# mihikamd/DP-GSAT

Hardware: AMD Instinct MI355X
Metric: million edges/s (attn+sample+aggregate fwd+bwd) (higher is better)
Workload: dtype f32

## Files before the change

dp_gsat_amd/_lib.py:

```python
from __future__ import annotations

import ctypes
import os
from ctypes import c_char_p, c_double, c_float, c_int, c_int32, c_int64, c_size_t, c_uint64, c_void_p

import torch

_HERE = os.path.dirname(os.path.abspath(__file__))
LIB_PATH = os.path.join(_HERE, "libgsat_hip.so")

P, I64, I32, F32, F64, SZ, INT, U64 = c_void_p, c_int64, c_int32, c_float, c_double, c_size_t, c_int, c_uint64

SIGNATURES = {
    "gsat_abi_version": (INT, []),
    "gsat_seed_next": (INT, [P, P, P]),
    "gsat_last_error": (c_char_p, []),
    "gsat_csr_workspace_bytes": (SZ, [I64, I64]),
    "gsat_rev_workspace_bytes": (SZ, [I64]),
    "gsat_build_csr": (INT, [P, P, I64, I64, P, P, P, P, P, SZ, P]),
    "gsat_reverse_edge_perm": (INT, [P, I64, I64, P, P, P, SZ, P]),
    "gsat_reverse_edge_perm_csr": (INT, [P, P, P, P, P, P, P, P, I64, I64, P, P, P]),
    "gsat_segment_ptr": (INT, [P, I64, I64, P, P, P]),
    "gsat_gather_i64": (INT, [P, I64, P, I64, P, P]),
    "gsat_row_chunks_workspace_bytes": (SZ, [I64]),
# ... 29 lines not shown
    "gsat_bn_apply_fwd": (INT, [P, P, P, P, P, I64, I64, INT, P, F32, U64, P, P, P]),
    "gsat_bn_local_bwd_sums": (INT, [P, P, P, P, P, P, I64, I64, INT, F32, U64, P, P, P, P, P]),
    "gsat_bn_apply_bwd": (INT, [P, P, P, P, P, P, P, P, I64, P, I64, I64, INT, F32, U64, P, P, P, P]),
    "gsat_relu_dropout_fwd": (INT, [P, I64, I64, F32, U64, P, P, P]),
    "gsat_relu_dropout_bwd": (INT, [P, P, I64, I64, F32, P, P]),
    "gsat_colsum_workspace_floats": (SZ, [I64]),
    "gsat_colsum": (INT, [P, I64, I64, P, P, P]),
    "gsat_embsum_fwd": (INT, [P, P, INT, P, I64, I64, P, P]),
    "gsat_onehot_rows": (INT, [P, P, INT, I64, I64, P, P]),
    "gsat_gemm_workspace_floats": (SZ, [INT, I64, I64, I64]),
    "gsat_gemm_plan": (INT, [INT, INT, INT, I64, I64, I64, INT, INT, I64, P]),
    "gsat_gemm_f32": (INT, [INT, INT, I64, I64, I64, P, I64, P, I64, P, I64, P, INT, P, SZ, P]),
    "gsat_gemm_bf16x3": (INT, [INT, INT, I64, I64, I64, P, I64, P, I64, P, I64, P, INT, P, SZ, P]),
    "gsat_gemm_wgrad_plan": (INT, [I64, I64, I64, P]),
    "gsat_gemm_wgrad_x3": (INT, [I64, I64, I64, P, I64, P, I64, P, I64, INT, P, SZ, P]),
    "gsat_attn_fwd_workspace_bytes": (SZ, [P]),
    "gsat_attn_fwd_kind": (I32, [P]),
    "gsat_attn_bwd_workspace_bytes": (SZ, [P]),
    "gsat_attn_fwd": (INT, [P, P]),
    "gsat_attn_bwd": (INT, [P, P, P]),
    "gsat_instance_norm_fwd": (INT, [P, P, P, P, I64, I64, I64, P, P, P]),
    "gsat_instance_norm_bwd": (INT, [P, P, P, P, P, P, I64, I64, I64, P, P, P]),
    "gsat_philox_keep_mask": (INT, [U64, I32, I64, I64, F32, P, P]),
    "gsat_philox_noise": (INT, [U64, I64, P, P]),
    "gsat_sample_fwd": (INT, [P, P, INT, F32, F32, I64, P, P]),
    "gsat_sample_bwd": (INT, [P, P, F32, I64, P, P]),
    "gsat_gumbel_sigmoid_philox": (INT, [P, I64, F32, F32, U64, P, P, P]),
    "gsat_philox_gumbel_noise": (INT, [U64, I64, P, P]),
    "gsat_lift_fwd": (INT, [P, P, P, I64, P, P]),
    "gsat_lift_bwd": (INT, [P, P, P, P, P, P, P, P, I64, P, P]),
# ... 129 lines not shown
```

dp_gsat_amd/csrc/attn.hip:

```cpp
#include "common.h"
#include "attn_fused.h"
#include <cstdlib>

namespace gsat {

constexpr float IN_EPS = 1e-5f;
constexpr int SB = 256;
#ifndef GSAT_SB_LANES
#define GSAT_SB_LANES 16
#endif
constexpr int SB_LANES = GSAT_SB_LANES;
constexpr int SB_SLOTS = SB / SB_LANES;
constexpr int SB_RC = 2;

struct GemmWs { float* ptr; size_t floats; };
static int gemm_rm(hipStream_t stream, bool ta, bool tb, int64_t M, int64_t N, int64_t K, const float* A, int64_t lda, const float* B,
                   int64_t ldb, float beta, float* C, int64_t ldc, GemmWs ws = {nullptr, 0}, bool split_ok = false, SlabJob* defer = nullptr) {
    const char* env = getenv("GSAT_ATTN_BWD_SPLIT");
    const bool bwd_split = !(env && atoi(env) == 0);
    if (ta && !tb && split_ok && bwd_split) return gemm_wgrad(stream, M, N, K, A, lda, B, ldb, C, ldc, beta != 0.f, ws.ptr, ws.floats, defer);
    return gemm_f32(stream, ta, tb, M, N, K, A, lda, B, ldb, C, ldc, nullptr, beta != 0.f, ws.ptr, ws.floats, split_ok && bwd_split, defer);
}

template <bool EDGE>
struct PreAct {
    const float* P; const float* Q; const float* bias; const int32_t* src; const int32_t* dst; int C;
    __device__ __forceinline__ float4 load(int row, int c) const {
        float4 b = bias ? ld4(bias + c) : f4zero();
        float4 v;
        if (EDGE) {
            float4 p = ld4(P + (size_t)src[row] * C + c);
            float4 q = ld4(Q + (size_t)dst[row] * C + c);
            v = make_float4(p.x + q.x, p.y + q.y, p.z + q.z, p.w + q.w);
        } else {
            v = ld4(P + (size_t)row * C + c);
        }
// ... 845 lines not shown
    if (Z > 1) {
        const unsigned cb = (unsigned)ceil_div(G * C2, 256);
        k_zcombine<<<cb, 256, 0, stream>>>(zp1, a->seg_ptr, (int)G, Z, C2, 1, S1);
        k_zcombine<<<cb, 256, 0, stream>>>(zp2, a->seg_ptr, (int)G, Z, C2, 1, S2);
        k_zcombine<<<cb, 256, 0, stream>>>(zp3, a->seg_ptr, (int)G, Z, C2, 0, dw3p);
    }
    GSAT_LAUNCH_CHECK();
    if (!(merged && part_ok) && (rc = colsum(stream, dw3p, G, C2, gr->dW3, scratch))) return rc;
    if (Z > 1) {
        k_dh2<<<ew_blocks(M * (C2 / 4)), 256, 0, stream>>>(a->h2, a->b2, a->row_seg, mean2, rstd2, a->mask2, SeedRef{a->seed, a->seed_dev}, a->p_drop, a->training,
                                                           a->W3, dz, S1, S2, M, C2, dh2);
        GSAT_LAUNCH_CHECK();
    }
    if (dual_gemm_ok(1, M, C2, C1, C1)) {
        if ((rc = dual_gemm(stream, 1, M, C2, C1, C1, dh2, C2, a->a1, C1, a->W2, C1, da1, C1, 0, gr->dW2, C1, dws, dws_bytes))) return rc;
    } else {
        if ((rc = gemm_rm(stream, true, false, C2, C1, M, dh2, C2, a->a1, C1, 0.f, gr->dW2, C1, gws, true, &jobs[0]))) return rc;
        if ((rc = gemm_rm(stream, false, false, M, C1, C2, dh2, C2, a->W2, C1, 0.f, da1, C1, GemmWs{nullptr, 0}, true))) return rc;
    }
    if (Z == 1) {
        if (a->edge_mode) {
            PreAct<true> pre1{a->P, a->Q, a->b1, a->src, a->dst, C1};
            k_l1_bwd_stats<true, true><<<g1, SB, 0, stream>>>(da1, a->a1, a->seg_ptr, a->seg_order, sc, C1, S1p, S2p, pre1, mean1, rstd1);
        } else {
            PreAct<false> pre1{a->P, nullptr, a->b1, nullptr, nullptr, C1};
            k_l1_bwd_stats<true, false><<<g1, SB, 0, stream>>>(da1, a->a1, a->seg_ptr, a->seg_order, sc, C1, S1p, S2p, pre1, mean1, rstd1);
        }
    } else {
        k_l1_bwd_stats<false, false><<<g1, SB, 0, stream>>>(da1, a->a1, a->seg_ptr, a->seg_order, sc, C1, zp1, zp2);
    }
// ... 19 lines not shown
            if ((rc = dual_gemm(stream, 2, N, C1, H, H, dQ, C1, a->emb, H, a->W1 + H, 2 * H, gr->demb, H, 1, gr->dW1 + H, 2 * H, dws, dws_bytes))) return rc;
        } else {
        if ((rc = gemm_rm(stream, false, false, N, H, C1, dP, C1, a->W1, 2 * H, 0.f, gr->demb, H, GemmWs{nullptr, 0}, true))) return rc;
        if ((rc = gemm_rm(stream, false, false, N, H, C1, dQ, C1, a->W1 + H, 2 * H, 1.f, gr->demb, H, GemmWs{nullptr, 0}, true))) return rc;
        if ((rc = gemm_rm(stream, true, false, C1, H, N, dP, C1, a->emb, H, 0.f, gr->dW1, 2 * H, gws1, true, &jobs[1]))) return rc;
        if ((rc = gemm_rm(stream, true, false, C1, H, N, dQ, C1, a->emb, H, 0.f, gr->dW1 + H, 2 * H, gws1b, true, &jobs[2]))) return rc;
        }
    } else {
        if (Z > 1) {
            PreAct<false> pre{a->P, nullptr, a->b1, nullptr, nullptr, C1};
            k_dh1<false><<<ew_blocks(M * (C1 / 4)), 256, 0, stream>>>(pre, a->row_seg, mean1, rstd1, a->a1, sc, S1p, S2p, M, da1);
            GSAT_LAUNCH_CHECK();
        }
        if (dual_gemm_ok(2, N, C1, H, H)) {
            if ((rc = dual_gemm(stream, 2, N, C1, H, H, da1, C1, a->emb, H, a->W1, H, gr->demb, H, 0, gr->dW1, H, dws, dws_bytes))) return rc;
        } else {
        if ((rc = gemm_rm(stream, false, false, N, H, C1, da1, C1, a->W1, H, 0.f, gr->demb, H, GemmWs{nullptr, 0}, true))) return rc;
        if ((rc = gemm_rm(stream, true, false, C1, H, N, da1, C1, a->emb, H, 0.f, gr->dW1, H, gws1, true, &jobs[1]))) return rc;
        }
    }
    return slab_reduce_jobs(stream, jobs, 3);
}

int gsat_instance_norm_fwd(const float* x, const int32_t* seg_ptr, const int32_t* seg_order, const int32_t* row_seg, int64_t M,
                           int64_t G, int64_t C, float* y, float* stats, void* stream_) {
    hipStream_t stream = (hipStream_t)stream_;
    GSAT_REQUIRE(M >= 0 && G >= 0 && C > 0 && C % 4 == 0 && M < (1ll << 31), GSAT_ERR_UNSUPPORTED, "gsat_instance_norm_fwd: C must be a positive multiple of 4");
    if (M == 0 || G == 0) return GSAT_OK;
    GSAT_REQUIRE(x && seg_ptr && row_seg && y && stats, GSAT_ERR_ARG, "gsat_instance_norm_fwd: null pointer");
    float* mean = stats;
// ... 44 lines not shown
```

dp_gsat_amd/csrc/common.h:

```cpp
#pragma once
#include <cstring>
#include <cstdint>
#include <cstdio>
#include <cstdarg>
#include <hip/hip_runtime.h>

#include "../../include/gsat_hip.h"

namespace gsat {

void set_error(const char* fmt, ...);
const char* get_error();

#define GSAT_CHECK_HIP(expr)                                                                  \
    do {                                                                                      \
        hipError_t _e = (expr);                                                               \
        if (_e != hipSuccess) {                                                               \
            gsat::set_error("%s:%d: %s -> %s", __FILE__, __LINE__, #expr, hipGetErrorString(_e)); \
            return GSAT_ERR_HIP;                                                              \
        }                                                                                     \
    } while (0)

#define GSAT_REQUIRE(cond, code, ...)                                                         \
    do {                                                                                      \
// ... 23 lines not shown
    }
    bool ok() const { return base != nullptr && off <= cap; }
};

struct SlabJob { const float* ws; int nslab; size_t slab; int M, N; int64_t ldc; int accumulate; float* out; };
int gemm_f32(hipStream_t stream, bool a_t, bool b_t, int64_t M, int64_t N, int64_t K, const float* A, int64_t lda, const float* B,
             int64_t ldb, float* C, int64_t ldc, const float* bias, bool accumulate, float* ws, size_t ws_floats, bool allow_split = false,
             SlabJob* defer = nullptr);
int slab_reduce_jobs(hipStream_t stream, const SlabJob* jobs, int n);
size_t gemm_workspace_floats(int64_t M, int64_t N, int64_t K, bool reduce_rows);
struct WgradPlan { int eligible, S, rows; size_t ws_floats; };
WgradPlan wgrad_plan(int64_t Mo, int64_t No, int64_t K);
size_t gemm_wgrad_workspace_floats(int64_t Mo, int64_t No, int64_t K);
int gemm_wgrad(hipStream_t stream, int64_t Mo, int64_t No, int64_t K, const float* A, int64_t lda, const float* B, int64_t ldb, float* C,
               int64_t ldc, bool accumulate, float* ws, size_t ws_floats, SlabJob* defer = nullptr);

int aggr_sum_fwd_impl(hipStream_t stream, const float* x, const float* self_rows, const float* att, const float* edge_emb,
                      const int32_t* rowptr, const int32_t* col, const int32_t* eid, int64_t N, int64_t E, int64_t H, float self_coef,
                      float* out, const int32_t* chunk_ptr, float* partial);

#ifdef __HIPCC__
constexpr int WAVE = 64;

template <int CTRL> __device__ __forceinline__ float dpp_add(float v) {
    const int t = __builtin_amdgcn_update_dpp(0, __builtin_bit_cast(int, v), CTRL, 0xF, 0xF, true);
    return v + __builtin_bit_cast(float, t);
}

template <int WIDTH> __device__ __forceinline__ float group_sum(float v) {
    if constexpr ((WIDTH & (WIDTH - 1)) == 0) {
// ... 111 lines not shown
```

dp_gsat_amd/csrc/gemm.hip:

```cpp
#include "common.h"
#include "pna_math.h"
#include <cstdlib>

namespace gsat {

typedef float f32x16 __attribute__((ext_vector_type(16)));

constexpr int GK = 32, GT = 256;
constexpr int LD_KC = 129;
constexpr int LD_KM = 132;

struct StageKC { float4 v[4]; };
template <int ROWS>
__device__ __forceinline__ void load_kcontig(StageKC& s, const float* __restrict__ X, int64_t ld, int r0, int R, int k0, int K, int t) {
    const int kq = (t & 7) * 4;
#pragma unroll
    for (int p = 0; p < ROWS / 32; ++p) {
        const int r = r0 + (t >> 3) + 32 * p;
        s.v[p] = (r < R && k0 + kq < K) ? ld4(X + (size_t)r * ld + k0 + kq) : f4zero();
    }
}
template <int ROWS>
__device__ __forceinline__ void store_kcontig(const StageKC& s, float* __restrict__ L, int t) {
    const int kq = (t & 7) * 4;
// ... 13 lines not shown
#pragma unroll
    for (int p = 0; p < GK / KPP; ++p) {
        const int k = k0 + t / QPR + KPP * p;
        s.v[p] = (k < K && c0 + cq < Ccols) ? ld4(X + (size_t)k * ld + c0 + cq) : f4zero();
    }
}
template <int COLS>
__device__ __forceinline__ void store_kmajor(const StageKC& s, float* __restrict__ L, int t) {
    constexpr int QPR = COLS / 4, KPP = GT / QPR;
    const int cq = (t % QPR) * 4;
#pragma unroll
    for (int p = 0; p < GK / KPP; ++p) st4(L + (t / QPR + KPP * p) * LD_KM + cq, s.v[p]);
}

__device__ int GEMM_XCD_REMAP_ON = 1;
__device__ __forceinline__ void gemm_tile_coords(int& bx, int& by, int& bz) {
    const unsigned gx = gridDim.x, gy = gridDim.y, total = gx * gy * gridDim.z;
    const unsigned L = (blockIdx.z * gy + blockIdx.y) * gx + blockIdx.x;
    if (!GEMM_XCD_REMAP_ON) { bx = blockIdx.x; by = blockIdx.y; bz = blockIdx.z; return; }
    const unsigned q = total >> 3, r = total & 7, xcd = L & 7, i = L >> 3;
    const unsigned t = (xcd < r ? xcd * (q + 1) : r * (q + 1) + (xcd - r) * q) + i;
    bx = (int)(t % gx); by = (int)((t / gx) % gy); bz = (int)(t / (gx * gy));
}

template <bool A_T, bool B_T, int TM, int TN>
__global__ __launch_bounds__(GT) void k_gemm_f32(const float* __restrict__ A, int64_t lda, const float* __restrict__ B, int64_t ldb,
                                                 float* __restrict__ C, int64_t ldc, int M, int N, int K, int k_per_split,
                                                 const float* __restrict__ bias, int accumulate, size_t slab_stride) {
    constexpr int GM = 64 * TM, GN = 64 * TN;
    constexpr int LDA = A_T ? LD_KM : LD_KC, LDB = B_T ? LD_KC : LD_KM;
    constexpr int EP_LD = 36;
    static_assert(GK * LDA + GK * LDB >= 4 * 32 * EP_LD, "epilogue staging must fit in the operand images");
    __shared__ __attribute__((aligned(16))) float lds[GK * LDA + GK * LDB];
    float* const As = lds;
    float* const Bs = lds + GK * LDA;
    const int t = threadIdx.x, lane = t & 63, wave = t >> 6;
    const int wm = wave >> 1, wn = wave & 1;
// ... 415 lines not shown
                if (m0 + WS_ROWS <= M) {
#pragma unroll
                    for (int r = 0; r < 16; ++r) crow[(size_t)((r & 3) + 8 * (r >> 2)) * ldc] = acc[r] + bv;
                } else {
#pragma unroll
                    for (int r = 0; r < 16; ++r)
                        if (m0 + 4 * h + (r & 3) + 8 * (r >> 2) < M) crow[(size_t)((r & 3) + 8 * (r >> 2)) * ldc] = acc[r] + bv;
                }
            }
        }
        if (KS > 1) __syncthreads();
        float* tmp = cur; cur = nxt; nxt = tmp;
    }
}

template <bool B_T, int KSTEPS, int NQ>
__global__ __launch_bounds__(WS_THREADS, 2) void k_gemm_ws_x3(const float* __restrict__ A, int64_t lda, const float* __restrict__ B, int64_t ldb,
                                                             float* __restrict__ C, int64_t ldc, int M, int N, int K, int NB, int accumulate, int tiles) {
    extern __shared__ __attribute__((aligned(16))) unsigned char wx_lds[];
    const int RS = 2 * K + 16;
    const int PLANE = WS_ROWS * RS;
    unsigned char* const buf0 = wx_lds;
    unsigned char* const buf1 = wx_lds + 2 * PLANE;
    const int t = threadIdx.x, lane = t & 63, wave = t >> 6;
    const int cb = wave % NB, ks = wave / NB, KS = 8 / NB;
    const int c = lane & 31, h = lane >> 5;
    const int n0 = blockIdx.y * (NB * 32) + cb * 32;
    const int kw0 = ks * (KSTEPS * 16);
    bf16x8 bh[KSTEPS], bl[KSTEPS];
    {
        const int col = min(n0 + c, N - 1);
#pragma unroll
        for (int s_ = 0; s_ < KSTEPS; ++s_) {
            float v[8];
            const int k0 = kw0 + 16 * s_ + 8 * h;
            if (B_T) {
                const float4 v0 = ld4(B + (size_t)col * ldb + k0), v1 = ld4(B + (size_t)col * ldb + k0 + 4);
                v[0] = v0.x; v[1] = v0.y; v[2] = v0.z; v[3] = v0.w; v[4] = v1.x; v[5] = v1.y; v[6] = v1.z; v[7] = v1.w;
            } else {
#pragma unroll
                for (int j = 0; j < 8; ++j) v[j] = B[(size_t)(k0 + j) * ldb + col];
            }
            uint4 H = make_uint4(pack_bf16(v[0], v[1]), pack_bf16(v[2], v[3]), pack_bf16(v[4], v[5]), pack_bf16(v[6], v[7]));
            uint4 L = make_uint4(pack_bf16(v[0] - bf16_hi(v[0]), v[1] - bf16_hi(v[1])), pack_bf16(v[2] - bf16_hi(v[2]), v[3] - bf16_hi(v[3])),
                                 pack_bf16(v[4] - bf16_hi(v[4]), v[5] - bf16_hi(v[5])), pack_bf16(v[6] - bf16_hi(v[6]), v[7] - bf16_hi(v[7])));
            bh[s_] = *reinterpret_cast<bf16x8*>(&H);
            bl[s_] = *reinterpret_cast<bf16x8*>(&L);
        }
    }
    const int K4 = K >> 2;
    int srow[NQ], soff[NQ];
#pragma unroll
    for (int p = 0; p < NQ; ++p) {
        const int idx = t + p * WS_THREADS;
        srow[p] = idx / K4;
        soff[p] = 4 * (idx % K4);
    }
    float4 st[NQ];
    auto gload = [&](int tile) {
        const int m0 = tile * WS_ROWS;
#pragma unroll
        for (int p = 0; p < NQ; ++p) st[p] = ld4(A + (size_t)min(m0 + srow[p], M - 1) * lda + soff[p]);
    };
    auto lstore = [&](unsigned char* dst) {
#pragma unroll
        for (int p = 0; p < NQ; ++p) {
            const float4 v = st[p];
            const uint2 H = make_uint2(pack_bf16(v.x, v.y), pack_bf16(v.z, v.w));
            const uint2 L = make_uint2(pack_bf16(v.x - bf16_hi(v.x), v.y - bf16_hi(v.y)), pack_bf16(v.z - bf16_hi(v.z), v.w - bf16_hi(v.w)));
            *reinterpret_cast<uint2*>(dst + srow[p] * RS + soff[p] * 2) = H;
            *reinterpret_cast<uint2*>(dst + PLANE + srow[p] * RS + soff[p] * 2) = L;
        }
    };
    int tile = blockIdx.x;
    if (tile < tiles) { gload(tile); lstore(buf0); }
    __builtin_amdgcn_s_waitcnt(0x0F70);
    __syncthreads();
    unsigned char* cur = buf0;
    unsigned char* nxt = buf1;
    const bool col_ok = n0 + c < N;
    for (; tile < tiles; tile += gridDim.x) {
        const int ntile = tile + gridDim.x;
        if (ntile < tiles) gload(ntile);
        f32x16 acc;
#pragma unroll
        for (int r = 0; r < 16; ++r) acc[r] = 0.f;
        const unsigned char* arow = cur + c * RS + (kw0 + 8 * h) * 2;
#pragma unroll
        for (int s_ = 0; s_ < KSTEPS; ++s_) {
            const bf16x8 ah = *reinterpret_cast<const bf16x8*>(arow + 32 * s_);
            const bf16x8 al = *reinterpret_cast<const bf16x8*>(arow + PLANE + 32 * s_);
            acc = __builtin_amdgcn_mfma_f32_32x32x16_bf16(al, bl[s_], acc, 0, 0, 0);
            acc = __builtin_amdgcn_mfma_f32_32x32x16_bf16(al, bh[s_], acc, 0, 0, 0);
            acc = __builtin_amdgcn_mfma_f32_32x32x16_bf16(ah, bl[s_], acc, 0, 0, 0);
            acc = __builtin_amdgcn_mfma_f32_32x32x16_bf16(ah, bh[s_], acc, 0, 0, 0);
        }
        float* const xch = reinterpret_cast<float*>(cur);
        if (KS > 1) {
            __syncthreads();
            if (ks > 0) {
                float* part = xch + ((ks - 1) * NB + cb) * 1024;
#pragma unroll
                for (int r = 0; r < 16; ++r) part[r * 64 + lane] = acc[r];
            }
        }
        if (ntile < tiles) lstore(nxt);
        __syncthreads();
        if (ks == 0) {
            if (KS > 1) {
                for (int s2 = 1; s2 < KS; ++s2) {
                    const float* part = xch + ((s2 - 1) * NB + cb) * 1024;
#pragma unroll
                    for (int r = 0; r < 16; ++r) acc[r] += part[r * 64 + lane];
                }
            }
            const int m0 = tile * WS_ROWS;
            float* crow = C + (size_t)(m0 + 4 * h) * ldc + n0 + c;
            if (col_ok) {
#pragma unroll
                for (int r = 0; r < 16; ++r) {
                    const int rr = (r & 3) + 8 * (r >> 2);
                    if (m0 + 4 * h + rr < M) {
                        if (accumulate & 2) __builtin_nontemporal_store(acc[r], crow + (size_t)rr * ldc);
                        else crow[(size_t)rr * ldc] = (accumulate & 1) ? crow[(size_t)rr * ldc] + acc[r] : acc[r];
                    }
                }
            }
        }
        if (KS > 1) __syncthreads();
        unsigned char* tmp = cur; cur = nxt; nxt = tmp;
    }
}

__global__ void k_slab_reduce(const float* __restrict__ slabs, int nslab, size_t slab_stride, int M, int N, int64_t ldc,
                              int accumulate, float* __restrict__ out) {
    const int64_t i = (int64_t)blockIdx.x * blockDim.x + threadIdx.x;
    if (i >= (int64_t)M * N) return;
    const float* p0 = slabs + i;
    float a[8] = {0.f, 0.f, 0.f, 0.f, 0.f, 0.f, 0.f, 0.f};
    int s = 0;
    for (; s + 8 <= nslab; s += 8) {
#pragma unroll
        for (int j = 0; j < 8; ++j) a[j] += p0[(size_t)(s + j) * slab_stride];
    }
    for (int j = 0; s < nslab; ++s, ++j) a[j] += p0[(size_t)s * slab_stride];
    const float acc = ((a[0] + a[1]) + (a[2] + a[3])) + ((a[4] + a[5]) + (a[6] + a[7]));
// ... 148 lines not shown
    const int64_t NB = (N > 256 ? 256 : N) / 32;
    if (NB != 1 && NB != 2 && NB != 4 && NB != 8) return false;
    const int64_t KS = 8 / NB, Kw = K / KS;
    if (Kw % 16 != 0) return false;
    const int64_t st = Kw / 16;
    if (st != 2 && st != 4 && st != 8) return false;
    if ((KS - 1) * NB * 4096 > 2 * WS_ROWS * (2 * K + 16)) return false;
    *nb = (int)NB; *ksteps = (int)st;
    return true;
}
static bool wsx3_applicable(int64_t M, int64_t N, int64_t K) {
    static const int on = getenv("GSAT_GEMM_WSX3") ? atoi(getenv("GSAT_GEMM_WSX3")) : 1;
    int nb, st;
    return on && M >= 8192 && M < (1ll << 31) - 64 && wsx3_geometry(N, K, &nb, &st);
}
template <bool B_T, int KSTEPS, int NQ>
static int wsx3_launch(hipStream_t stream, dim3 grid, size_t lds, const float* A, int64_t lda, const float* B, int64_t ldb, float* C, int64_t ldc,
                       int M, int N, int K, int nb, int accumulate, int tiles) {
    static size_t allowed = 64 * 1024;
    if (lds > allowed) {
        GSAT_CHECK_HIP(hipFuncSetAttribute((const void*)k_gemm_ws_x3<B_T, KSTEPS, NQ>, hipFuncAttributeMaxDynamicSharedMemorySize, (int)lds));
        allowed = lds;
    }
    k_gemm_ws_x3<B_T, KSTEPS, NQ><<<grid, WS_THREADS, lds, stream>>>(A, lda, B, ldb, C, ldc, M, N, K, nb, accumulate, tiles);
    GSAT_LAUNCH_CHECK();
    return GSAT_OK;
}
static int gemm_wsx3(hipStream_t stream, bool b_t, int64_t M, int64_t N, int64_t K, const float* A, int64_t lda, const float* B, int64_t ldb,
                     float* C, int64_t ldc, bool accumulate, int nb, int st) {
    const int tiles = (int)ceil_div(M, WS_ROWS);
    const size_t lds = (size_t)4 * WS_ROWS * (2 * K + 16);
    const int nq = (int)(K / 64);
    const int per_cu = (2 * lds <= 150 * 1024 && st * 8 + nq * 9 <= 84) ? 2 : 1;
    const int chunks = (int)ceil_div(N, 256);
    const dim3 grid((unsigned)std::min<int64_t>(tiles, std::max<int64_t>(1, (int64_t)256 * per_cu / chunks)), (unsigned)chunks);
    static const int nt_mode = getenv("GSAT_GEMM_NT") ? atoi(getenv("GSAT_GEMM_NT")) : 1;
    const int acc_flag = (accumulate ? 1 : 0) | ((nt_mode && !accumulate && (size_t)M * N * 4 >= ((size_t)64 << 20)) ? 2 : 0);
#define XGO(BT, S, Q) return wsx3_launch<BT, S, Q>(stream, grid, lds, A, lda, B, ldb, C, ldc, (int)M, (int)N, (int)K, nb, acc_flag, tiles)
#define XQ(BT, S) do { switch (nq) { case 1: XGO(BT, S, 1); case 2: XGO(BT, S, 2); case 4: XGO(BT, S, 4); case 8: XGO(BT, S, 8); default: break; } } while (0)
#define XS(BT) do { switch (st) { case 2: XQ(BT, 2); break; case 4: XQ(BT, 4); break; default: XQ(BT, 8); break; } } while (0)
    if (b_t) XS(true); else XS(false);
#undef XS
#undef XQ
#undef XGO
    GSAT_REQUIRE(false, GSAT_ERR_UNSUPPORTED, "gemm_wsx3: K = %lld is not 64, 128, 256 or 512", (long long)K);
}

enum { GEMM_TILE_F32 = 0, GEMM_TILE_X3 = 1, GEMM_WS_F32 = 2, GEMM_WS_X3 = 3 };
struct GemmPlan {
    int family;
    int tm, tn;
    int splits;
// ... 106 lines not shown
    }
    for (int q = m; q <= 4; ++q) J.first[q] = blocks;
    if (!blocks) return GSAT_OK;
    if (wide == 4) k_slab_reduce_jobs<16><<<blocks, 256, 0, stream>>>(J);
    else if (wide == 2) k_slab_reduce_jobs<8><<<blocks, 256, 0, stream>>>(J);
    else k_slab_reduce_jobs<4><<<blocks, 256, 0, stream>>>(J);
    GSAT_LAUNCH_CHECK();
    return GSAT_OK;
}

constexpr int WG_T = 512, WG_TILE = 128;
constexpr int WG_PLANE = (GK / 8) * WG_TILE * 16;
constexpr int WG_BUF = 4 * WG_PLANE;
constexpr int WG_MIN_SLABS = 8;

__global__ __launch_bounds__(WG_T) void k_wgrad_x3(const float* A, int64_t lda, const float* B, int64_t ldb, float* ws, int Mo, int No, int K,
                                                   int rows_per) {
    constexpr int EP_LD = 36;
    static_assert(2 * WG_BUF >= 8 * 32 * EP_LD * 4, "epilogue staging must fit in the operand planes");
    __shared__ __attribute__((aligned(16))) unsigned char lds[2 * WG_BUF];
    const int t = threadIdx.x, lane = t & 63, wave = t >> 6;
    int bx, by, bz;
    gemm_tile_coords(bx, by, bz);
    const int m0 = by * WG_TILE, n0 = bx * WG_TILE;
    const int kbeg = bz * rows_per, kend = min(K, kbeg + rows_per);
    const int nslab = (kend - kbeg + GK - 1) / GK;
    const int ts = t & 255, cp = (ts & 63) * 2, k8 = ts >> 6;
    const bool stage_b = t >= 256;
    const float* const src = stage_b ? B + n0 + cp : A + m0 + cp;
    const int64_t ld = stage_b ? ldb : lda;
    const int plane0 = stage_b ? 2 * WG_PLANE : 0;
    auto gload = [&](StageKM& s, int slab) {
        const int kb = kbeg + slab * GK + k8 * 8;
#pragma unroll
        for (int j = 0; j < 8; ++j) s.v[j] = *reinterpret_cast<const float2*>(src + (size_t)min(kb + j, kend - 1) * ld);
    };
    auto lstore = [&](StageKM& s, int slab, unsigned char* buf) {
        const int kb = kbeg + slab * GK + k8 * 8;
// ... 64 lines not shown
    const int prow = lane >> 3, pcol = (lane & 7) * 4;
#pragma unroll
    for (int j = 0; j < 2; ++j) {
#pragma unroll
        for (int r = 0; r < 16; ++r) patch[((r & 3) + 8 * (r >> 2) + 4 * kh) * EP_LD + r32] = acc[j][r];
        __builtin_amdgcn_wave_barrier();
        const int col = n0 + wn * 64 + j * 32 + pcol;
#pragma unroll
        for (int p = 0; p < 4; ++p) {
            const int rr = prow + 8 * p;
            st4(Cb + (size_t)(m0 + wm * 32 + rr) * No + col, ld4(patch + rr * EP_LD + pcol));
        }
        __builtin_amdgcn_wave_barrier();
    }
}

static int device_cus() {
    static const int n = [] {
        int dev = 0, v = 0;
        if (hipGetDevice(&dev) != hipSuccess || hipDeviceGetAttribute(&v, hipDeviceAttributeMultiprocessorCount, dev) != hipSuccess || v <= 0) {
            (void)hipGetLastError();
            v = 256;
        }
        return v;
    }();
    return n;
}

WgradPlan wgrad_plan(int64_t Mo, int64_t No, int64_t K) {
    WgradPlan p{};
// ... 18 lines not shown

int gemm_wgrad(hipStream_t stream, int64_t Mo, int64_t No, int64_t K, const float* A, int64_t lda, const float* B, int64_t ldb, float* C,
               int64_t ldc, bool accumulate, float* ws, size_t ws_floats, SlabJob* defer) {
    const WgradPlan p = wgrad_plan(Mo, No, K);
    if (!p.eligible) return gemm_f32(stream, true, false, Mo, No, K, A, lda, B, ldb, C, ldc, nullptr, accumulate, ws, ws_floats, true, defer);
    if (defer) defer->nslab = 0;
    xcd_switch_once();
    GSAT_REQUIRE(A && B && C && lda >= Mo && ldb >= No && ldc >= No && lda % 4 == 0 && ldb % 4 == 0 && ldc % 4 == 0, GSAT_ERR_ARG, "gemm_wgrad: bad argument");
    GSAT_REQUIRE(((uintptr_t)A % 16 == 0) && ((uintptr_t)B % 16 == 0) && ((uintptr_t)C % 16 == 0) && ((uintptr_t)ws % 16 == 0), GSAT_ERR_ARG,
                 "gemm_wgrad: operands, output and workspace must be 16-byte aligned");
    GSAT_REQUIRE(ws && ws_floats >= p.ws_floats, GSAT_ERR_WORKSPACE, "gemm_wgrad: workspace too small");
    const dim3 grid((unsigned)(No / WG_TILE), (unsigned)(Mo / WG_TILE), (unsigned)p.S);
    k_wgrad_x3<<<grid, WG_T, 0, stream>>>(A, lda, B, ldb, ws, (int)Mo, (int)No, (int)K, p.rows);
    GSAT_LAUNCH_CHECK();
    const SlabJob job{ws, p.S, (size_t)Mo * No, (int)Mo, (int)No, ldc, accumulate ? 1 : 0, C};
    if (defer) { *defer = job; return GSAT_OK; }
    return slab_reduce_jobs(stream, &job, 1);
}

int pna_post_fwd(hipStream_t stream, const PnaVirt& pv, int64_t Nrows, const float* W, int64_t ldw, const float* bias, int64_t Ho, float* out, int64_t ldo) {
    const int64_t K = (int64_t)pv.NAGG * 2 * pv.H;
    GSAT_REQUIRE(pv.H % 32 == 0 && Ho % 4 == 0 && ldw % 4 == 0 && ldo % 4 == 0 && Nrows < (1ll << 31), GSAT_ERR_UNSUPPORTED, "gsat_pna_post_fwd: H must be a multiple of 32, Ho of 4");
    GSAT_REQUIRE(((uintptr_t)W % 16 == 0) && ((uintptr_t)out % 16 == 0) && (!bias || (uintptr_t)bias % 16 == 0) && ((uintptr_t)pv.x % 16 == 0) && ((uintptr_t)pv.aggj % 16 == 0),
                 GSAT_ERR_ARG, "gsat_pna_post_fwd: operands must be 16-byte aligned");
    if (Nrows <= 0 || Ho <= 0) return GSAT_OK;
    xcd_switch_once();
    const int tn = Ho > 64 ? 2 : 1;
    dim3 grid((unsigned)ceil_div(Ho, 64 * tn), (unsigned)ceil_div(Nrows, 128), 1);
    if (tn == 2) k_gemm_bf16x3<false, true, 2, 2, 1><<<grid, GT, 0, stream>>>(nullptr, 0, W, ldw, out, ldo, (int)Nrows, (int)Ho, (int)K, (int)K, bias, 0, 0, pv);
    else k_gemm_bf16x3<false, true, 2, 1, 1><<<grid, GT, 0, stream>>>(nullptr, 0, W, ldw, out, ldo, (int)Nrows, (int)Ho, (int)K, (int)K, bias, 0, 0, pv);
// ... 79 lines not shown

int gsat_gemm_wgrad_plan(int64_t Mo, int64_t No, int64_t K, int32_t* plan) {
    GSAT_REQUIRE(plan && Mo > 0 && No > 0 && K > 0, GSAT_ERR_ARG, "gsat_gemm_wgrad_plan: bad argument");
    const WgradPlan p = wgrad_plan(Mo, No, K);
    GSAT_REQUIRE(p.ws_floats <= (size_t)INT32_MAX, GSAT_ERR_UNSUPPORTED, "gsat_gemm_wgrad_plan: workspace of %zu floats does not fit int32", p.ws_floats);
    const int32_t v[4] = {p.eligible, p.S, p.rows, (int32_t)p.ws_floats};
    memcpy(plan, v, sizeof(v));
    return GSAT_OK;
}

int gsat_gemm_wgrad_x3(int64_t Mo, int64_t No, int64_t K, const float* A, int64_t lda, const float* B, int64_t ldb, float* C, int64_t ldc,
                       int accumulate, float* workspace, size_t workspace_floats, void* stream) {
    return gemm_wgrad((hipStream_t)stream, Mo, No, K, A, lda, B, ldb, C, ldc, accumulate != 0, workspace, workspace_floats);
}

int gsat_gemm_plan(int allow_split, int a_t, int b_t, int64_t M, int64_t N, int64_t K, int has_bias, int accumulate, int64_t ldb, int32_t* plan) {
    GSAT_REQUIRE(plan && M > 0 && N > 0 && K > 0, GSAT_ERR_ARG, "gsat_gemm_plan: bad argument");
    GSAT_REQUIRE(ldb % 4 == 0 && (a_t ? M % 4 == 0 : K % 4 == 0) && (b_t ? K % 4 == 0 : N % 4 == 0), GSAT_ERR_UNSUPPORTED,
                 "gsat_gemm_plan: contiguous extents and leading dimensions must be multiples of 4 (M=%lld N=%lld K=%lld)", (long long)M, (long long)N, (long long)K);
    const GemmPlan p = gemm_plan(allow_split != 0, a_t != 0, b_t != 0, M, N, K, has_bias != 0, accumulate != 0, ldb);
    GSAT_REQUIRE(!(has_bias && p.splits > 1), GSAT_ERR_UNSUPPORTED, "gsat_gemm_plan: bias with split-K");
    const int32_t v[8] = {p.family, p.tm, p.tn, p.splits, p.reduce, p.nb, p.kr, p.nq};
    memcpy(plan, v, sizeof(v));
    return GSAT_OK;
}

}
```

include/gsat_hip.h:

```cpp
#ifndef GSAT_HIP_H
#define GSAT_HIP_H

#include <stddef.h>
#include <stdint.h>

#ifdef __cplusplus
extern "C" {
#endif

#define GSAT_ABI_VERSION 4

#define GSAT_OK 0
#define GSAT_ERR_HIP (-1)
#define GSAT_ERR_ARG (-2)
#define GSAT_ERR_WORKSPACE (-3)
#define GSAT_ERR_UNSUPPORTED (-4)
#define GSAT_ERR_BLAS (-5)

int gsat_abi_version(void);

int gsat_seed_next(uint64_t* state, uint64_t* out, void* stream);
const char* gsat_last_error(void);


// ... 156 lines not shown
                     void* stream);


size_t gsat_gemm_workspace_floats(int a_t, int64_t M, int64_t N, int64_t K);
int gsat_gemm_plan(int allow_split, int a_t, int b_t, int64_t M, int64_t N, int64_t K, int has_bias, int accumulate,
                   int64_t ldb, int32_t* plan);
int gsat_gemm_f32(int a_t, int b_t, int64_t M, int64_t N, int64_t K, const float* A, int64_t lda,
                  const float* B, int64_t ldb, float* C, int64_t ldc, const float* bias, int accumulate,
                  float* workspace, size_t workspace_floats, void* stream);
int gsat_gemm_bf16x3(int a_t, int b_t, int64_t M, int64_t N, int64_t K, const float* A, int64_t lda,
                     const float* B, int64_t ldb, float* C, int64_t ldc, const float* bias, int accumulate,
                     float* workspace, size_t workspace_floats, void* stream);
int gsat_gemm_wgrad_plan(int64_t Mo, int64_t No, int64_t K, int32_t* plan);
int gsat_gemm_wgrad_x3(int64_t Mo, int64_t No, int64_t K, const float* A, int64_t lda, const float* B, int64_t ldb,
                       float* C, int64_t ldc, int accumulate, float* workspace, size_t workspace_floats, void* stream);


typedef struct gsat_attn_args {
    int64_t M, N, G;
    int32_t H, C1, C2;
    int32_t edge_mode;
    int32_t training;
    float p_drop;
    uint64_t seed;
    const int32_t* src;
    const int32_t* dst;
    const int32_t* seg_ptr;
    const int32_t* seg_order;
    const int32_t* row_seg;
    const float *W1, *b1, *W2, *b2, *W3, *b3;
// ... 229 lines not shown
```

Baseline: 132.5.

## Co-schedule weight-grad and data-grad GEMMs in one paired kernel launch

```diff
diff --git a/dp_gsat_amd/_lib.py b/dp_gsat_amd/_lib.py
--- a/dp_gsat_amd/_lib.py
+++ b/dp_gsat_amd/_lib.py
@@ -67,6 +67,8 @@
     "gsat_gemm_bf16x3": (INT, [INT, INT, I64, I64, I64, P, I64, P, I64, P, I64, P, INT, P, SZ, P]),
     "gsat_gemm_wgrad_plan": (INT, [I64, I64, I64, P]),
     "gsat_gemm_wgrad_x3": (INT, [I64, I64, I64, P, I64, P, I64, P, I64, INT, P, SZ, P]),
+    "gsat_gemm_pair_plan": (INT, [I64, I64, I64, I64, P]),
+    "gsat_gemm_pair_x3": (INT, [I64, I64, I64, I64, P, I64, P, I64, P, I64, P, I64, P, I64, INT, P, SZ, P]),
     "gsat_attn_fwd_workspace_bytes": (SZ, [P]),
     "gsat_attn_fwd_kind": (I32, [P]),
     "gsat_attn_bwd_workspace_bytes": (SZ, [P]),
diff --git a/dp_gsat_amd/csrc/attn.hip b/dp_gsat_amd/csrc/attn.hip
--- a/dp_gsat_amd/csrc/attn.hip
+++ b/dp_gsat_amd/csrc/attn.hip
@@ -20,6 +20,10 @@
     const bool bwd_split = !(env && atoi(env) == 0);
     if (ta && !tb && split_ok && bwd_split) return gemm_wgrad(stream, M, N, K, A, lda, B, ldb, C, ldc, beta != 0.f, ws.ptr, ws.floats, defer);
     return gemm_f32(stream, ta, tb, M, N, K, A, lda, B, ldb, C, ldc, nullptr, beta != 0.f, ws.ptr, ws.floats, split_ok && bwd_split, defer);
+}
+static bool pair_ok(int64_t R, int64_t Cg, int64_t Co, int64_t Cy) {
+    const char* env = getenv("GSAT_ATTN_BWD_SPLIT");
+    return !(env && atoi(env) == 0) && gemm_pair_plan(R, Cg, Co, Cy).paired;
 }
 
 template <bool EDGE>
@@ -895,6 +899,8 @@
     }
     if (dual_gemm_ok(1, M, C2, C1, C1)) {
         if ((rc = dual_gemm(stream, 1, M, C2, C1, C1, dh2, C2, a->a1, C1, a->W2, C1, da1, C1, 0, gr->dW2, C1, dws, dws_bytes))) return rc;
+    } else if (pair_ok(M, C2, C1, C1)) {
+        if ((rc = gemm_pair_x3(stream, M, C2, C1, C1, dh2, C2, a->W2, C1, da1, C1, a->a1, C1, gr->dW2, C1, false, gws.ptr, gws.floats, &jobs[0]))) return rc;
     } else {
         if ((rc = gemm_rm(stream, true, false, C2, C1, M, dh2, C2, a->a1, C1, 0.f, gr->dW2, C1, gws, true, &jobs[0]))) return rc;
         if ((rc = gemm_rm(stream, false, false, M, C1, C2, dh2, C2, a->W2, C1, 0.f, da1, C1, GemmWs{nullptr, 0}, true))) return rc;
@@ -944,6 +950,8 @@
         }
         if (dual_gemm_ok(2, N, C1, H, H)) {
             if ((rc = dual_gemm(stream, 2, N, C1, H, H, da1, C1, a->emb, H, a->W1, H, gr->demb, H, 0, gr->dW1, H, dws, dws_bytes))) return rc;
+        } else if (pair_ok(N, C1, H, H)) {
+            if ((rc = gemm_pair_x3(stream, N, C1, H, H, da1, C1, a->W1, H, gr->demb, H, a->emb, H, gr->dW1, H, false, gws1.ptr, gws1.floats, &jobs[1]))) return rc;
         } else {
         if ((rc = gemm_rm(stream, false, false, N, H, C1, da1, C1, a->W1, H, 0.f, gr->demb, H, GemmWs{nullptr, 0}, true))) return rc;
         if ((rc = gemm_rm(stream, true, false, C1, H, N, da1, C1, a->emb, H, 0.f, gr->dW1, H, gws1, true, &jobs[1]))) return rc;
diff --git a/dp_gsat_amd/csrc/common.h b/dp_gsat_amd/csrc/common.h
--- a/dp_gsat_amd/csrc/common.h
+++ b/dp_gsat_amd/csrc/common.h
@@ -61,6 +61,11 @@
 size_t gemm_wgrad_workspace_floats(int64_t Mo, int64_t No, int64_t K);
 int gemm_wgrad(hipStream_t stream, int64_t Mo, int64_t No, int64_t K, const float* A, int64_t lda, const float* B, int64_t ldb, float* C,
                int64_t ldc, bool accumulate, float* ws, size_t ws_floats, SlabJob* defer = nullptr);
+struct PairPlan { int paired, wgrad_blocks, dgrad_blocks, lds_bytes; };
+PairPlan gemm_pair_plan(int64_t R, int64_t Cg, int64_t Co, int64_t Cy);
+int gemm_pair_x3(hipStream_t stream, int64_t R, int64_t Cg, int64_t Co, int64_t Cy, const float* G, int64_t ldg, const float* W, int64_t ldw,
+                 float* OUT, int64_t ldo, const float* Y, int64_t ldy, float* DW, int64_t lddw, bool accumulate, float* ws, size_t ws_floats,
+                 SlabJob* defer = nullptr);
 
 int aggr_sum_fwd_impl(hipStream_t stream, const float* x, const float* self_rows, const float* att, const float* edge_emb,
                       const int32_t* rowptr, const int32_t* col, const int32_t* eid, int64_t N, int64_t E, int64_t H, float self_coef,
diff --git a/dp_gsat_amd/csrc/gemm.hip b/dp_gsat_amd/csrc/gemm.hip
--- a/dp_gsat_amd/csrc/gemm.hip
+++ b/dp_gsat_amd/csrc/gemm.hip
@@ -51,13 +51,17 @@
 }
 
 __device__ int GEMM_XCD_REMAP_ON = 1;
+__device__ __forceinline__ void gemm_tile_coords(unsigned L, unsigned gx, unsigned gy, unsigned gz, int& bx, int& by, int& bz) {
+    const unsigned total = gx * gy * gz;
+    unsigned t = L;
+    if (GEMM_XCD_REMAP_ON) {
+        const unsigned q = total >> 3, r = total & 7, xcd = L & 7, i = L >> 3;
+        t = (xcd < r ? xcd * (q + 1) : r * (q + 1) + (xcd - r) * q) + i;
+    }
+    bx = (int)(t % gx); by = (int)((t / gx) % gy); bz = (int)(t / (gx * gy));
+}
 __device__ __forceinline__ void gemm_tile_coords(int& bx, int& by, int& bz) {
-    const unsigned gx = gridDim.x, gy = gridDim.y, total = gx * gy * gridDim.z;
-    const unsigned L = (blockIdx.z * gy + blockIdx.y) * gx + blockIdx.x;
-    if (!GEMM_XCD_REMAP_ON) { bx = blockIdx.x; by = blockIdx.y; bz = blockIdx.z; return; }
-    const unsigned q = total >> 3, r = total & 7, xcd = L & 7, i = L >> 3;
-    const unsigned t = (xcd < r ? xcd * (q + 1) : r * (q + 1) + (xcd - r) * q) + i;
-    bx = (int)(t % gx); by = (int)((t / gx) % gy); bz = (int)(t / (gx * gy));
+    gemm_tile_coords((blockIdx.z * gridDim.y + blockIdx.y) * gridDim.x + blockIdx.x, gridDim.x, gridDim.y, gridDim.z, bx, by, bz);
 }
 
 template <bool A_T, bool B_T, int TM, int TN>
@@ -503,10 +507,11 @@
     }
 }
 
-template <bool B_T, int KSTEPS, int NQ>
-__global__ __launch_bounds__(WS_THREADS, 2) void k_gemm_ws_x3(const float* __restrict__ A, int64_t lda, const float* __restrict__ B, int64_t ldb,
-                                                             float* __restrict__ C, int64_t ldc, int M, int N, int K, int NB, int accumulate, int tiles) {
-    extern __shared__ __attribute__((aligned(16))) unsigned char wx_lds[];
+template <bool B_T, int KSTEPS, int NQ, bool KFIX = false>
+__device__ __forceinline__ void gemm_ws_x3_body(unsigned char* wx_lds, int bx, int by, int gx, const float* __restrict__ A, int64_t lda,
+                                                const float* __restrict__ B, int64_t ldb, float* __restrict__ C, int64_t ldc, int M, int N, int K_,
+                                                int NB_, int accumulate, int tiles) {
+    const int K = KFIX ? 64 * NQ : K_, NB = KFIX ? 2 * KSTEPS / NQ : NB_;
     const int RS = 2 * K + 16;
     const int PLANE = WS_ROWS * RS;
     unsigned char* const buf0 = wx_lds;
@@ -514,7 +519,7 @@
     const int t = threadIdx.x, lane = t & 63, wave = t >> 6;
     const int cb = wave % NB, ks = wave / NB, KS = 8 / NB;
     const int c = lane & 31, h = lane >> 5;
-    const int n0 = blockIdx.y * (NB * 32) + cb * 32;
+    const int n0 = by * (NB * 32) + cb * 32;
     const int kw0 = ks * (KSTEPS * 16);
     bf16x8 bh[KSTEPS], bl[KSTEPS];
     {
@@ -545,31 +550,38 @@
         srow[p] = idx / K4;
         soff[p] = 4 * (idx % K4);
     }
-    float4 st[NQ];
-    auto gload = [&](int tile) {
+    constexpr bool HALVES = KFIX && NQ == 4 && KSTEPS == 8;
+    constexpr int NS = HALVES ? NQ / 2 : NQ;
+    float4 st[NS];
+    auto gload = [&](int tile, int half = 0) {
         const int m0 = tile * WS_ROWS;
 #pragma unroll
-        for (int p = 0; p < NQ; ++p) st[p] = ld4(A + (size_t)min(m0 + srow[p], M - 1) * lda + soff[p]);
+        for (int p = 0; p < NS; ++p)
+            st[p] = ld4(A + (size_t)min(m0 + srow[p + half * NS], M - 1) * lda + soff[p + half * NS]);
     };
-    auto lstore = [&](unsigned char* dst) {
-#pragma unroll
-        for (int p = 0; p < NQ; ++p) {
+    auto lstore = [&](unsigned char* dst, int half = 0) {
+#pragma unroll
+        for (int p = 0; p < NS; ++p) {
             const float4 v = st[p];
+            const int o = srow[p + half * NS] * RS + soff[p + half * NS] * 2;
             const uint2 H = make_uint2(pack_bf16(v.x, v.y), pack_bf16(v.z, v.w));
             const uint2 L = make_uint2(pack_bf16(v.x - bf16_hi(v.x), v.y - bf16_hi(v.y)), pack_bf16(v.z - bf16_hi(v.z), v.w - bf16_hi(v.w)));
-            *reinterpret_cast<uint2*>(dst + srow[p] * RS + soff[p] * 2) = H;
-            *reinterpret_cast<uint2*>(dst + PLANE + srow[p] * RS + soff[p] * 2) = L;
+            *reinterpret_cast<uint2*>(dst + o) = H;
+            *reinterpret_cast<uint2*>(dst + PLANE + o) = L;
         }
     };
-    int tile = blockIdx.x;
-    if (tile < tiles) { gload(tile); lstore(buf0); }
+    int tile = bx;
+    if (tile < tiles) {
+        gload(tile); lstore(buf0);
+        if (HALVES) { gload(tile, 1); lstore(buf0, 1); }
+    }
     __builtin_amdgcn_s_waitcnt(0x0F70);
     __syncthreads();
     unsigned char* cur = buf0;
     unsigned char* nxt = buf1;
     const bool col_ok = n0 + c < N;
-    for (; tile < tiles; tile += gridDim.x) {
-        const int ntile = tile + gridDim.x;
+    for (; tile < tiles; tile += gx) {
+        const int ntile = tile + gx;
         if (ntile < tiles) gload(ntile);
         f32x16 acc;
 #pragma unroll
@@ -583,6 +595,7 @@
             acc = __builtin_amdgcn_mfma_f32_32x32x16_bf16(al, bh[s_], acc, 0, 0, 0);
             acc = __builtin_amdgcn_mfma_f32_32x32x16_bf16(ah, bl[s_], acc, 0, 0, 0);
             acc = __builtin_amdgcn_mfma_f32_32x32x16_bf16(ah, bh[s_], acc, 0, 0, 0);
+            if (HALVES && s_ == KSTEPS / 2 - 1 && ntile < tiles) { lstore(nxt); gload(ntile, 1); }
         }
         float* const xch = reinterpret_cast<float*>(cur);
         if (KS > 1) {
@@ -593,7 +606,7 @@
                 for (int r = 0; r < 16; ++r) part[r * 64 + lane] = acc[r];
             }
         }
-        if (ntile < tiles) lstore(nxt);
+        if (ntile < tiles) lstore(nxt, HALVES ? 1 : 0);
         __syncthreads();
         if (ks == 0) {
             if (KS > 1) {
@@ -619,6 +632,12 @@
         if (KS > 1) __syncthreads();
         unsigned char* tmp = cur; cur = nxt; nxt = tmp;
     }
+}
+template <bool B_T, int KSTEPS, int NQ>
+__global__ __launch_bounds__(WS_THREADS, 2) void k_gemm_ws_x3(const float* __restrict__ A, int64_t lda, const float* __restrict__ B, int64_t ldb,
+                                                             float* __restrict__ C, int64_t ldc, int M, int N, int K, int NB, int accumulate, int tiles) {
+    extern __shared__ __attribute__((aligned(16))) unsigned char wx_lds[];
+    gemm_ws_x3_body<B_T, KSTEPS, NQ>(wx_lds, (int)blockIdx.x, (int)blockIdx.y, (int)gridDim.x, A, lda, B, ldb, C, ldc, M, N, K, NB, accumulate, tiles);
 }
 
 __global__ void k_slab_reduce(const float* __restrict__ slabs, int nslab, size_t slab_stride, int M, int N, int64_t ldc,
@@ -797,6 +816,10 @@
     int nb, st;
     return on && M >= 8192 && M < (1ll << 31) - 64 && wsx3_geometry(N, K, &nb, &st);
 }
+static int wsx3_out_flag(bool accumulate, int64_t M, int64_t N) {
+    static const int nt_mode = getenv("GSAT_GEMM_NT") ? atoi(getenv("GSAT_GEMM_NT")) : 1;
+    return (accumulate ? 1 : 0) | ((nt_mode && !accumulate && (size_t)M * N * 4 >= ((size_t)64 << 20)) ? 2 : 0);
+}
 template <bool B_T, int KSTEPS, int NQ>
 static int wsx3_launch(hipStream_t stream, dim3 grid, size_t lds, const float* A, int64_t lda, const float* B, int64_t ldb, float* C, int64_t ldc,
                        int M, int N, int K, int nb, int accumulate, int tiles) {
@@ -817,8 +840,7 @@
     const int per_cu = (2 * lds <= 150 * 1024 && st * 8 + nq * 9 <= 84) ? 2 : 1;
     const int chunks = (int)ceil_div(N, 256);
     const dim3 grid((unsigned)std::min<int64_t>(tiles, std::max<int64_t>(1, (int64_t)256 * per_cu / chunks)), (unsigned)chunks);
-    static const int nt_mode = getenv("GSAT_GEMM_NT") ? atoi(getenv("GSAT_GEMM_NT")) : 1;
-    const int acc_flag = (accumulate ? 1 : 0) | ((nt_mode && !accumulate && (size_t)M * N * 4 >= ((size_t)64 << 20)) ? 2 : 0);
+    const int acc_flag = wsx3_out_flag(accumulate, M, N);
 #define XGO(BT, S, Q) return wsx3_launch<BT, S, Q>(stream, grid, lds, A, lda, B, ldb, C, ldc, (int)M, (int)N, (int)K, nb, acc_flag, tiles)
 #define XQ(BT, S) do { switch (nq) { case 1: XGO(BT, S, 1); case 2: XGO(BT, S, 2); case 4: XGO(BT, S, 4); case 8: XGO(BT, S, 8); default: break; } } while (0)
 #define XS(BT) do { switch (st) { case 2: XQ(BT, 2); break; case 4: XQ(BT, 4); break; default: XQ(BT, 8); break; } } while (0)
@@ -955,14 +977,13 @@
 constexpr int WG_BUF = 4 * WG_PLANE;
 constexpr int WG_MIN_SLABS = 8;
 
-__global__ __launch_bounds__(WG_T) void k_wgrad_x3(const float* A, int64_t lda, const float* B, int64_t ldb, float* ws, int Mo, int No, int K,
-                                                   int rows_per) {
+__device__ __forceinline__ void wgrad_x3_body(unsigned char* lds, unsigned L, unsigned gx, unsigned gy, unsigned gz, const float* A, int64_t lda,
+                                              const float* B, int64_t ldb, float* ws, int Mo, int No, int K, int rows_per) {
     constexpr int EP_LD = 36;
     static_assert(2 * WG_BUF >= 8 * 32 * EP_LD * 4, "epilogue staging must fit in the operand planes");
-    __shared__ __attribute__((aligned(16))) unsigned char lds[2 * WG_BUF];
     const int t = threadIdx.x, lane = t & 63, wave = t >> 6;
     int bx, by, bz;
-    gemm_tile_coords(bx, by, bz);
+    gemm_tile_coords(L, gx, gy, gz, bx, by, bz);
     const int m0 = by * WG_TILE, n0 = bx * WG_TILE;
     const int kbeg = bz * rows_per, kend = min(K, kbeg + rows_per);
     const int nslab = (kend - kbeg + GK - 1) / GK;
@@ -1057,6 +1078,27 @@
         __builtin_amdgcn_wave_barrier();
     }
 }
+__global__ __launch_bounds__(WG_T) void k_wgrad_x3(const float* A, int64_t lda, const float* B, int64_t ldb, float* ws, int Mo, int No, int K,
+                                                   int rows_per) {
+    __shared__ __attribute__((aligned(16))) unsigned char lds[2 * WG_BUF];
+    wgrad_x3_body(lds, (blockIdx.z * gridDim.y + blockIdx.y) * gridDim.x + blockIdx.x, gridDim.x, gridDim.y, gridDim.z, A, lda, B, ldb, ws, Mo, No, K,
+                  rows_per);
+}
+
+struct PairWgrad { const float* Y; int64_t ldy; float* ws; int Cy, rows_per; unsigned gx, gy, gz; };
+template <int KSTEPS, int NQ>
+__global__ __launch_bounds__(WG_T, 4) void k_pair_x3(const float* G, int64_t ldg, const float* W, int64_t ldw, float* OUT, int64_t ldo, int R, int Cg,
+                                                     int Co, int NB, int out_flag, int tiles, unsigned dgx, unsigned both, const PairWgrad wg) {
+    static_assert(WG_T == WS_THREADS, "both bodies run on the same workgroup size");
+    extern __shared__ __attribute__((aligned(16))) unsigned char pair_lds[];
+    const unsigned L = blockIdx.x, nw = wg.gx * wg.gy * wg.gz;
+    unsigned role, V;
+    if (L < 2 * both) { role = (L >> 3) & 1; V = ((L >> 4) << 3) | (L & 7); }
+    else if (L - 2 * both < nw - both) { role = 0; V = L - both; }
+    else { role = 1; V = L - nw; }
+    if (role == 0) wgrad_x3_body(pair_lds, V, wg.gx, wg.gy, wg.gz, G, ldg, wg.Y, wg.ldy, wg.ws, Cg, wg.Cy, R, wg.rows_per);
+    else gemm_ws_x3_body<false, KSTEPS, NQ, KSTEPS == 8 || NQ == 2>(pair_lds, (int)(V % dgx), (int)(V / dgx), (int)dgx, G, ldg, W, ldw, OUT, ldo, R, Co, Cg, NB, out_flag, tiles);
+}
 
 static int device_cus() {
     static const int n = [] {
@@ -1105,6 +1147,76 @@
     k_wgrad_x3<<<grid, WG_T, 0, stream>>>(A, lda, B, ldb, ws, (int)Mo, (int)No, (int)K, p.rows);
     GSAT_LAUNCH_CHECK();
     const SlabJob job{ws, p.S, (size_t)Mo * No, (int)Mo, (int)No, ldc, accumulate ? 1 : 0, C};
+    if (defer) { *defer = job; return GSAT_OK; }
+    return slab_reduce_jobs(stream, &job, 1);
+}
+
+PairPlan gemm_pair_plan(int64_t R, int64_t Cg, int64_t Co, int64_t Cy) {
+    static const int on = getenv("GSAT_GEMM_PAIR") ? atoi(getenv("GSAT_GEMM_PAIR")) : 1;
+    PairPlan pp{};
+    if (R <= 0 || Cg <= 0 || Co <= 0 || Cy <= 0 || Cg % 4 != 0 || Co % 4 != 0) return pp;
+    const GemmPlan g = gemm_plan(true, false, false, R, Co, Cg, false, false, Co);
+    const WgradPlan w = wgrad_plan(Cg, Cy, R);
+    if (!on || g.family != GEMM_WS_X3 || !w.eligible) return pp;
+    const size_t lds = std::max<size_t>(2 * WG_BUF, (size_t)4 * WS_ROWS * (2 * Cg + 16));
+    if (2 * lds > (size_t)160 * 1024) return pp;
+    const int64_t chunks = ceil_div(Co, 256), tiles = ceil_div(R, WS_ROWS);
+    pp.paired = 1;
+    pp.wgrad_blocks = (int)((Cg / WG_TILE) * (Cy / WG_TILE) * w.S);
+    pp.dgrad_blocks = (int)(std::min<int64_t>(tiles, std::max<int64_t>(1, device_cus() / chunks)) * chunks);
+    pp.lds_bytes = (int)lds;
+    return pp;
+}
+
+template <int KSTEPS, int NQ>
+static int pair_launch(hipStream_t stream, unsigned blocks, size_t lds, const float* G, int64_t ldg, const float* W, int64_t ldw, float* OUT, int64_t ldo,
+                       int R, int Cg, int Co, int nb, int out_flag, int tiles, unsigned dgx, unsigned both, const PairWgrad& wg) {
+    static size_t allowed = 64 * 1024;
+    if (lds > allowed) {
+        GSAT_CHECK_HIP(hipFuncSetAttribute((const void*)k_pair_x3<KSTEPS, NQ>, hipFuncAttributeMaxDynamicSharedMemorySize, (int)lds));
+        allowed = lds;
+    }
+    k_pair_x3<KSTEPS, NQ><<<blocks, WG_T, lds, stream>>>(G, ldg, W, ldw, OUT, ldo, R, Cg, Co, nb, out_flag, tiles, dgx, both, wg);
+    GSAT_LAUNCH_CHECK();
+    return GSAT_OK;
+}
+
+int gemm_pair_x3(hipStream_t stream, int64_t R, int64_t Cg, int64_t Co, int64_t Cy, const float* G, int64_t ldg, const float* W, int64_t ldw,
+                 float* OUT, int64_t ldo, const float* Y, int64_t ldy, float* DW, int64_t lddw, bool accumulate, float* ws, size_t ws_floats,
+                 SlabJob* defer) {
+    const PairPlan pp = gemm_pair_plan(R, Cg, Co, Cy);
+    if (!pp.paired) {
+        const int rc = gemm_wgrad(stream, Cg, Cy, R, G, ldg, Y, ldy, DW, lddw, accumulate, ws, ws_floats, defer);
+        if (rc) return rc;
+        return gemm_f32(stream, false, false, R, Co, Cg, G, ldg, W, ldw, OUT, ldo, nullptr, false, nullptr, 0, true);
+    }
+    if (defer) defer->nslab = 0;
+    xcd_switch_once();
+    const WgradPlan w = wgrad_plan(Cg, Cy, R);
+    const GemmPlan g = gemm_plan(true, false, false, R, Co, Cg, false, false, Co);
+    GSAT_REQUIRE(G && W && OUT && Y && DW && ldg >= Cg && ldw >= Co && ldo >= Co && ldy >= Cy && lddw >= Cy, GSAT_ERR_ARG, "gemm_pair_x3: bad argument");
+    GSAT_REQUIRE(ldg % 4 == 0 && ldw % 4 == 0 && ldo % 4 == 0 && ldy % 4 == 0 && lddw % 4 == 0, GSAT_ERR_UNSUPPORTED,
+                 "gemm_pair_x3: leading dimensions must be multiples of 4");
+    GSAT_REQUIRE(((uintptr_t)G % 16 == 0) && ((uintptr_t)W % 16 == 0) && ((uintptr_t)OUT % 16 == 0) && ((uintptr_t)Y % 16 == 0) &&
+                 ((uintptr_t)DW % 16 == 0) && ((uintptr_t)ws % 16 == 0), GSAT_ERR_ARG, "gemm_pair_x3: operands, outputs and workspace must be 16-byte aligned");
+    GSAT_REQUIRE(ws && ws_floats >= w.ws_floats, GSAT_ERR_WORKSPACE, "gemm_pair_x3: workspace too small");
+    const int tiles = (int)ceil_div(R, WS_ROWS);
+    const unsigned chunks = (unsigned)ceil_div(Co, 256), dgx = (unsigned)pp.dgrad_blocks / chunks;
+    const unsigned both = (unsigned)std::min(pp.wgrad_blocks, pp.dgrad_blocks) / 8 * 8;
+    const PairWgrad wg{Y, ldy, ws, (int)Cy, w.rows, (unsigned)(Cy / WG_TILE), (unsigned)(Cg / WG_TILE), (unsigned)w.S};
+    const int out_flag = wsx3_out_flag(false, R, Co);
+    const unsigned blocks = (unsigned)(pp.wgrad_blocks + pp.dgrad_blocks);
+    int rc;
+#define PGO(S, Q) rc = pair_launch<S, Q>(stream, blocks, (size_t)pp.lds_bytes, G, ldg, W, ldw, OUT, ldo, (int)R, (int)Cg, (int)Co, g.nb, out_flag, tiles, dgx, both, wg)
+    if (g.kr == 8 && g.nq == 2) PGO(8, 2);
+    else if (g.kr == 4 && g.nq == 2) PGO(4, 2);
+    else if (g.kr == 8 && g.nq == 4) PGO(8, 4);
+    else if (g.kr == 4 && g.nq == 4) PGO(4, 4);
+    else if (g.kr == 2 && g.nq == 4) PGO(2, 4);
+    else GSAT_REQUIRE(false, GSAT_ERR_UNSUPPORTED, "gemm_pair_x3: no kernel for KSTEPS = %d, NQ = %d", g.kr, g.nq);
+#undef PGO
+    if (rc) return rc;
+    const SlabJob job{ws, w.S, (size_t)Cg * Cy, (int)Cg, (int)Cy, lddw, accumulate ? 1 : 0, DW};
     if (defer) { *defer = job; return GSAT_OK; }
     return slab_reduce_jobs(stream, &job, 1);
 }
@@ -1214,6 +1326,20 @@
     return gemm_wgrad((hipStream_t)stream, Mo, No, K, A, lda, B, ldb, C, ldc, accumulate != 0, workspace, workspace_floats);
 }
 
+int gsat_gemm_pair_plan(int64_t R, int64_t Cg, int64_t Co, int64_t Cy, int32_t* plan) {
+    GSAT_REQUIRE(plan && R > 0 && Cg > 0 && Co > 0 && Cy > 0, GSAT_ERR_ARG, "gsat_gemm_pair_plan: bad argument");
+    const PairPlan p = gemm_pair_plan(R, Cg, Co, Cy);
+    const int32_t v[4] = {p.paired, p.wgrad_blocks, p.dgrad_blocks, p.lds_bytes};
+    memcpy(plan, v, sizeof(v));
+    return GSAT_OK;
+}
+
+int gsat_gemm_pair_x3(int64_t R, int64_t Cg, int64_t Co, int64_t Cy, const float* G, int64_t ldg, const float* W, int64_t ldw, float* OUT, int64_t ldo,
+                      const float* Y, int64_t ldy, float* DW, int64_t lddw, int accumulate, float* workspace, size_t workspace_floats, void* stream) {
+    GSAT_REQUIRE(R > 0 && Cg > 0 && Co > 0 && Cy > 0, GSAT_ERR_ARG, "gsat_gemm_pair_x3: bad argument");
+    return gemm_pair_x3((hipStream_t)stream, R, Cg, Co, Cy, G, ldg, W, ldw, OUT, ldo, Y, ldy, DW, lddw, accumulate != 0, workspace, workspace_floats);
+}
+
 int gsat_gemm_plan(int allow_split, int a_t, int b_t, int64_t M, int64_t N, int64_t K, int has_bias, int accumulate, int64_t ldb, int32_t* plan) {
     GSAT_REQUIRE(plan && M > 0 && N > 0 && K > 0, GSAT_ERR_ARG, "gsat_gemm_plan: bad argument");
     GSAT_REQUIRE(ldb % 4 == 0 && (a_t ? M % 4 == 0 : K % 4 == 0) && (b_t ? K % 4 == 0 : N % 4 == 0), GSAT_ERR_UNSUPPORTED,
diff --git a/include/gsat_hip.h b/include/gsat_hip.h
--- a/include/gsat_hip.h
+++ b/include/gsat_hip.h
@@ -194,6 +194,10 @@
 int gsat_gemm_wgrad_plan(int64_t Mo, int64_t No, int64_t K, int32_t* plan);
 int gsat_gemm_wgrad_x3(int64_t Mo, int64_t No, int64_t K, const float* A, int64_t lda, const float* B, int64_t ldb,
                        float* C, int64_t ldc, int accumulate, float* workspace, size_t workspace_floats, void* stream);
+int gsat_gemm_pair_plan(int64_t R, int64_t Cg, int64_t Co, int64_t Cy, int32_t* plan);
+int gsat_gemm_pair_x3(int64_t R, int64_t Cg, int64_t Co, int64_t Cy, const float* G, int64_t ldg, const float* W, int64_t ldw,
+                      float* OUT, int64_t ldo, const float* Y, int64_t ldy, float* DW, int64_t lddw, int accumulate,
+                      float* workspace, size_t workspace_floats, void* stream);
 
 
 typedef struct gsat_attn_args {
```

Result: faster. 136.1, median of 6 (+2.6%).
